# LCSL/nys-koop-lqr

Hardware: AMD Instinct MI355X
Metric: Nyström-Koopman fits/sec (K_nm build + A,B,C solve), N=1e5 m=2000 d=384 (higher is better)
Workload: dtype f64

## Files before the change

### nys_koop_lqr_amd/csrc/nk_api.hip

```cpp
#include "nk_common.h"
#include "nk_plant.h"

#include <cmath>
#include <cstdarg>
#include <cstdio>
#include <cstring>
#include <chrono>
#include <cstdlib>
#include <algorithm>
#include <condition_variable>
#include <functional>
#include <mutex>
#include <set>
#include <thread>

namespace nk {

static thread_local std::string g_err;

void set_error(const char* fmt, ...) {
  char buf[1024];
  va_list ap;
  va_start(ap, fmt);
  vsnprintf(buf, sizeof(buf), fmt, ap);
// ... 293 lines not shown
    NK_TRY(launch_gemm(ctx, false, true, len, d, m, 1.0, phi, m, mdl->W, m + p, 0.0, out + r0 * ldo, ldo));
    if (p > 0)
      NK_TRY(launch_gemm(ctx, false, true, len, d, p, 1.0, Xaug + r0 * ldx + d, ldx, mdl->W + m, m + p, 1.0,
                         out + r0 * ldo, ldo));
  }
  arena_release(ctx, mk);
  return NK_OK;
}

struct HostTrace {
  bool on;
  std::chrono::steady_clock::time_point t0, last;
  HostTrace() : on(getenv("NYSKOOP_TRACE") != nullptr) { t0 = last = std::chrono::steady_clock::now(); }
  void mark(const char* what) {
    if (!on) return;
    auto now = std::chrono::steady_clock::now();
    fprintf(stderr, "[nk trace] %-28s +%8.3f ms (total %8.3f)\n", what,
            std::chrono::duration<double, std::milli>(now - last).count(),
            std::chrono::duration<double, std::milli>(now - t0).count());
    last = now;
  }
};

static float ev_ms(nk_ctx* ctx, int a, int b) {
  float ms = 0.f;
  (void)hipEventElapsedTime(&ms, ctx->ev[a], ctx->ev[b]);
  return ms;
}

}

using namespace nk;

extern "C" {

int nk_version(void) { return NK_ABI_VERSION; }

const char* nk_last_error(void) { return g_err.c_str(); }

int nk_device_count(void) {
  int n = 0;
  if (hipGetDeviceCount(&n) != hipSuccess) {
    (void)hipGetLastError();
    return 0;
  }
  return n;
}

int nk_create(int device, nk_ctx** out) {
  NK_REQUIRE(out != nullptr, "nk_create: null output pointer");
  *out = nullptr;
  int n = nk_device_count();
  if (n <= 0) {
    set_error("no HIP device visible: libnyskoop has no CPU fallback");
    return NK_ERR_NO_DEVICE;
  }
  NK_REQUIRE(device >= 0 && device < n, "nk_create: device %d out of range (0..%d)", device, n - 1);
  NK_HIP(hipSetDevice(device));
  hipDeviceProp_t prop;
  NK_HIP(hipGetDeviceProperties(&prop, device));
  if (strncmp(prop.gcnArchName, "gfx950", 6) != 0) {
    set_error("device %d is %s; libnyskoop is built for gfx950 (MI355X) only", device, prop.gcnArchName);
    return NK_ERR_NO_DEVICE;
  }
  nk_ctx* ctx = new nk_ctx();
  ctx->device = device;
  ctx->num_cu = prop.multiProcessorCount;
  int prio_lo = 0, prio_hi = 0;
  NK_HIP(hipDeviceGetStreamPriorityRange(&prio_lo, &prio_hi));
  const int prio_mid = (prio_lo - prio_hi >= 2) ? (prio_lo + prio_hi) / 2 : prio_hi;
  NK_HIP(hipStreamCreateWithPriority(&ctx->stream_main, hipStreamNonBlocking, prio_mid));
  NK_HIP(hipStreamCreateWithPriority(&ctx->stream_side, hipStreamNonBlocking, prio_lo));
  NK_HIP(hipStreamCreateWithPriority(&ctx->stream_prep, hipStreamNonBlocking, prio_hi));
  NK_HIP(hipStreamCreateWithFlags(&ctx->stream_copy, hipStreamNonBlocking));
  NK_HIP(hipStreamCreateWithPriority(&ctx->stream_la[0], hipStreamNonBlocking, prio_hi));
  NK_HIP(hipStreamCreateWithPriority(&ctx->stream_la[1], hipStreamNonBlocking, prio_mid));
  for (int q = 0; q < 2; ++q)
    for (int i = 0; i < 4; ++i) NK_HIP(hipEventCreateWithFlags(&ctx->ev_la[q][i], hipEventDisableTiming));
  ctx->stream = ctx->stream_main;
  ctx->cur_arena = &ctx->arena;
  NK_HIP(hipEventCreateWithFlags(&ctx->ev_fork, hipEventDisableTiming));
  NK_HIP(hipEventCreateWithFlags(&ctx->ev_join, hipEventDisableTiming));
  NK_HIP(hipEventCreateWithFlags(&ctx->ev_chain, hipEventDisableTiming));
  NK_HIP(hipMalloc(reinterpret_cast<void**>(&ctx->d_info), 256));
  ctx->d_piv = reinterpret_cast<unsigned long long*>(ctx->d_info + 16);
  NK_HIP(hipMalloc(reinterpret_cast<void**>(&ctx->d_scalars), 64 * sizeof(double)));
  NK_HIP(hipHostMalloc(reinterpret_cast<void**>(&ctx->h_scalars), 64 * sizeof(double), hipHostMallocMapped | hipHostMallocCoherent));
  NK_HIP(hipHostMalloc(reinterpret_cast<void**>(&ctx->h_info), 256, hipHostMallocMapped | hipHostMallocCoherent));
  ctx->h_piv = reinterpret_cast<unsigned long long*>(ctx->h_info + 16);
  for (int i = 0; i < 16; ++i) NK_HIP(hipEventCreate(&ctx->ev[i]));
  NK_HIP(hipEventCreateWithFlags(&ctx->ev_ext, hipEventDisableTiming));
  for (int i = 0; i < 8; ++i) NK_HIP(hipEventCreateWithFlags(&ctx->ev_up[i], hipEventDisableTiming));
  const char* km = getenv("NYSKOOP_KMAT");
  ctx->kmat_mode = (km && strcmp(km, "direct") == 0) ? 1 : 0;
  const char* st = getenv("NYSKOOP_STRICT_SPD");
  ctx->strict_spd = (st && atoi(st) != 0) ? 1 : 0;
  if (const char* rp = getenv("NYSKOOP_REFINE_PIVOT")) ctx->refine_pivot = atof(rp);
  if (const char* rs = getenv("NYSKOOP_REFINE_STEPS")) ctx->refine_steps = std::max(0, atoi(rs));
  {
    std::lock_guard<std::mutex> lk(g_reg_mu);
    g_ctxs.insert(ctx);
  }
  *out = ctx;
  return NK_OK;
}

static void destroy_ctx_unregistered(nk_ctx* ctx) {
  (void)hipSetDevice(ctx->device);
  if (tl_ctx == ctx) tl_ctx = nullptr;
  group_detach(ctx);
  (void)hipStreamSynchronize(ctx->stream_main);
  (void)hipStreamSynchronize(ctx->stream_side);
  (void)hipStreamSynchronize(ctx->stream_prep);
  (void)hipStreamSynchronize(ctx->stream_copy);
  for (int q = 0; q < 2; ++q) {
    if (ctx->stream_la[q]) { (void)hipStreamSynchronize(ctx->stream_la[q]); (void)hipStreamDestroy(ctx->stream_la[q]); }
    for (int i = 0; i < 4; ++i) if (ctx->ev_la[q][i]) (void)hipEventDestroy(ctx->ev_la[q][i]);
  }
  for (auto& c : ctx->arena.chunks) (void)hipFree(c.base);
  for (auto& c : ctx->arena_side.chunks) (void)hipFree(c.base);
  (void)hipEventDestroy(ctx->ev_fork);
  (void)hipEventDestroy(ctx->ev_join);
  if (ctx->ev_chain) (void)hipEventDestroy(ctx->ev_chain);
  if (ctx->ev_ext) (void)hipEventDestroy(ctx->ev_ext);
  for (int i = 0; i < 8; ++i) if (ctx->ev_up[i]) (void)hipEventDestroy(ctx->ev_up[i]);
  (void)hipStreamDestroy(ctx->stream_side);
  (void)hipStreamDestroy(ctx->stream_prep);
  (void)hipStreamDestroy(ctx->stream_copy);
  (void)hipFree(ctx->d_info);
  for (int i = 0; i < 2; ++i) if (ctx->d_flow[i]) (void)hipFree(ctx->d_flow[i]);
  (void)hipFree(ctx->d_scalars);
  if (ctx->d_zeros) (void)hipFree(ctx->d_zeros);
  if (ctx->h_stage) (void)hipHostFree(ctx->h_stage);
  (void)hipHostFree(ctx->h_scalars);
  (void)hipHostFree(ctx->h_info);
  for (int i = 0; i < 16; ++i) (void)hipEventDestroy(ctx->ev[i]);
  (void)hipStreamDestroy(ctx->stream_main);
  delete ctx;
}

int nk_destroy(nk_ctx* ctx) {
  if (!ctx) return NK_OK;
  {
    std::lock_guard<std::mutex> lk(g_reg_mu);
    if (g_ctxs.erase(ctx) == 0) return NK_OK;
  }
  destroy_ctx_unregistered(ctx);
  return NK_OK;
}

static int model_wait_unchecked(nk_model* mdl);
static void destroy_model_unregistered(nk_model* model, bool to_pool) {
  (void)model_wait_unchecked(model);
  if (to_pool) {
    pool_give(model->device, model->bytes, model->buf);
  } else {
    (void)hipSetDevice(model->device);
    (void)hipFree(model->buf);
  }
  delete model;
}

int nk_shutdown(void) {
  tl_ctx = nullptr;
  std::set<nk_ctx*> ctxs;
  std::set<nk_model*> models;
  std::set<void*> blocks;
  {
    std::lock_guard<std::mutex> lk(g_reg_mu);
    ctxs.swap(g_ctxs);
    models.swap(g_models);
    blocks.swap(g_host_blocks);
  }
  for (nk_ctx* c : ctxs) {
    (void)hipSetDevice(c->device);
    (void)hipStreamSynchronize(c->stream_main);
    (void)hipStreamSynchronize(c->stream_side);
    (void)hipStreamSynchronize(c->stream_prep);
    (void)hipStreamSynchronize(c->stream_copy);
  }
  for (nk_model* m : models) destroy_model_unregistered(m, false);
  for (nk_ctx* c : ctxs) destroy_ctx_unregistered(c);
  pool_drain();
  for (void* b : blocks) (void)hipHostFree(b);
  return NK_OK;
}

int nk_set_compute_dtype(nk_ctx* ctx, int dtype) {
  NK_REQUIRE(ctx != nullptr && (dtype == NK_DTYPE_F64 || dtype == NK_DTYPE_F32), "nk_set_compute_dtype: bad argument");
  ctx->compute_f32 = dtype == NK_DTYPE_F32 ? 1 : 0;
  return NK_OK;
}

int nk_set_strict_spd(nk_ctx* ctx, int strict) {
  NK_REQUIRE(ctx != nullptr && strict >= 0 && strict <= 2, "nk_set_strict_spd: bad argument");
  ctx->strict_spd = strict;
  return NK_OK;
}

int nk_set_refine(nk_ctx* ctx, double pivot_ratio, int32_t steps) {
  NK_REQUIRE(ctx != nullptr && pivot_ratio >= 0.0 && pivot_ratio <= 1.0 && steps >= 0 && steps <= 8, "nk_set_refine: bad argument");
  ctx->refine_pivot = pivot_ratio;
  ctx->refine_steps = steps;
  return NK_OK;
}

// ... 2112 lines not shown
```

### nys_koop_lqr_amd/csrc/nk_common.h

```cpp
#pragma once
#include <hip/hip_runtime.h>
#include <stdint.h>
#include <stddef.h>
#include <string>
#include <vector>

#include "nyskoop.h"
#include "nk_lockstep.h"

namespace nk {

void set_error(const char* fmt, ...);

#define NK_HIP(call)                                                                         \
  do {                                                                                       \
    hipError_t e_ = (call);                                                                  \
    if (e_ != hipSuccess) {                                                                  \
      nk::set_error("%s failed: %s (%s:%d)", #call, hipGetErrorString(e_), __FILE__, __LINE__); \
      return e_ == hipErrorOutOfMemory ? NK_ERR_OOM : NK_ERR_HIP;                            \
    }                                                                                        \
  } while (0)

#define NK_TRY(call)            \
  do {                          \
    int rc_ = (call);           \
    if (rc_ != NK_OK) return rc_; \
  } while (0)

#define NK_REQUIRE(cond, ...)     \
  do {                            \
    if (!(cond)) {                \
      nk::set_error(__VA_ARGS__); \
      return NK_ERR_BAD_ARG;      \
    }                             \
  } while (0)

struct ArenaChunk {
  char* base = nullptr;
  size_t cap = 0;
  size_t off = 0;
};
struct Arena {
  std::vector<ArenaChunk> chunks;
  int cur = 0;
};
struct ArenaMark {
  int chunk;
  size_t off;
};

}

struct nk_member_state;
struct nk_ctx {
  int device = 0;
  hipStream_t stream = nullptr;
  hipStream_t stream_main = nullptr;
  hipStream_t stream_side = nullptr;
  hipStream_t stream_copy = nullptr;
  hipStream_t stream_prep = nullptr;
  nk::Arena arena;
  nk::Arena arena_side;
  nk::Arena* cur_arena = nullptr;
  hipStream_t stream_la[2] = {nullptr, nullptr};
  hipEvent_t ev_la[2][4] = {};
  int compute_f32 = 0;
  hipEvent_t ev_fork = nullptr, ev_join = nullptr, ev_chain = nullptr;
  int* d_info = nullptr;
  unsigned long long* d_piv = nullptr;
  unsigned long long* h_piv = nullptr;
  double* d_scalars = nullptr;
  double* h_scalars = nullptr;
  int* h_info = nullptr;
  double* d_zeros = nullptr;
  hipEvent_t ev[16];
  int num_cu = 256;
  int kmat_mode = 0;
  double refine_pivot = 0.0;
  int refine_steps = 2;
  int strict_spd = 0;
  hipEvent_t ev_ext = nullptr;
  hipEvent_t ev_up[8] = {};
  nk_group* group = nullptr;
  nk_member_state* gstate = nullptr;
  int* d_flow[2] = {nullptr, nullptr};
  size_t flow_words[2] = {0, 0};
  bool spline_defer_svd = false;
  bool chol_flow_off = false;
  double* h_stage = nullptr;
  size_t h_stage_bytes = 0;
};

enum { NK_MODEL_NYSTROM = 0, NK_MODEL_SPLINE = 1 };
struct nk_model {
  int device = 0;
  int32_t m = 0, d = 0, p = 0;
  int32_t ktype = 0;
  double sigma0 = 0.0;
  double jitter = 0.0;
  double* buf = nullptr;
  size_t bytes = 0;
  double *A = nullptr, *B = nullptr, *C = nullptr, *W = nullptr, *S = nullptr, *Sinv = nullptr, *Z = nullptr,
         *winv = nullptr;
  bool has_ops = false;
  int32_t kind = 0;
  hipEvent_t ev_fetch = nullptr;
};

namespace nk {

struct SideScope {
  nk_ctx* c;
  hipStream_t s0;
  Arena* a0;
  explicit SideScope(nk_ctx* ctx, hipStream_t s = nullptr) : c(ctx), s0(ctx->stream), a0(ctx->cur_arena) {
    c->stream = s ? s : c->stream_side;
    c->cur_arena = &c->arena_side;
  }
  ~SideScope() {
    c->stream = s0;
    c->cur_arena = a0;
  }
};

struct ChainOnly {
  nk_ctx* c;
  bool b0;
  explicit ChainOnly(nk_ctx* ctx) : c(ctx), b0(ctx->chol_flow_off) { c->chol_flow_off = true; }
  ~ChainOnly() { c->chol_flow_off = b0; }
};

inline int info_base(const nk_ctx* c) { return c->stream != c->stream_main ? 2 : 0; }

__device__ __forceinline__ double exp_nonpos_ca() {
  double ca = __longlong_as_double(0x3e5ade156a5dcb37LL);
  asm volatile("" : "+v"(ca));
  return ca;
}
__device__ __forceinline__ double exp_nonpos(double x, double ca_v) {
  const double k = __builtin_rint(x * __longlong_as_double(0x3ff71547652b82feLL));
  double r = __builtin_fma(__longlong_as_double((long long)0xbfe62e42fefa39efULL), k, x);
  r = __builtin_fma(__longlong_as_double((long long)0xbc7abc9e3b39803fULL), k, r);
  double p;
#define NK_EXP_STEP(c) asm("v_fma_f64 %0, %1, %2, %3" : "=v"(p) : "v"(r), "v"(p), "s"(c))
  asm("v_fma_f64 %0, %1, %2, %3" : "=v"(p) : "v"(r), "v"(ca_v), "s"(__longlong_as_double(0x3e928af3fca7ab0cLL)));
  NK_EXP_STEP(__longlong_as_double(0x3ec71dee623fde64LL));
  NK_EXP_STEP(__longlong_as_double(0x3efa01997c89e6b0LL));
  NK_EXP_STEP(__longlong_as_double(0x3f2a01a014761f6eLL));
  NK_EXP_STEP(__longlong_as_double(0x3f56c16c1852b7b0LL));
  NK_EXP_STEP(__longlong_as_double(0x3f81111111122322LL));
  NK_EXP_STEP(__longlong_as_double(0x3fa55555555502a1LL));
  NK_EXP_STEP(__longlong_as_double(0x3fc5555555555511LL));
  NK_EXP_STEP(__longlong_as_double(0x3fe000000000000bLL));
#undef NK_EXP_STEP
  p = __builtin_fma(r, p, 1.0);
  p = __builtin_fma(r, p, 1.0);
  return x < -1075.0 ? 0.0 : ldexp(p, (int)k);
}
__device__ __forceinline__ double exp_nonpos(double x) { return exp_nonpos(x, exp_nonpos_ca()); }

__host__ __device__ __forceinline__ double log_pos(double x) {
#pragma clang fp contract(off)
  const double ln2_hi = 6.93147180369123816490e-01, ln2_lo = 1.90821492927058770002e-10;
  const double Lg1 = 6.666666666666735130e-01, Lg2 = 3.999999999940941908e-01, Lg3 = 2.857142874366239149e-01,
               Lg4 = 2.222219843214978396e-01, Lg5 = 1.818357216161805012e-01, Lg6 = 1.531383769920937332e-01,
               Lg7 = 1.479819860511658591e-01;
  uint64_t bits;
  __builtin_memcpy(&bits, &x, 8);
  int32_t hx = (int32_t)(bits >> 32);
  int k = 0;
  if (hx < 0x00100000) {
    x *= 1.80143985094819840000e+16;
    k -= 54;
    __builtin_memcpy(&bits, &x, 8);
    hx = (int32_t)(bits >> 32);
  }
  k += (hx >> 20) - 1023;
  hx &= 0x000fffff;
  const int32_t i = (hx + 0x95f64) & 0x100000;
  bits = ((uint64_t)(uint32_t)(hx | (i ^ 0x3ff00000)) << 32) | (bits & 0xffffffffULL);
  __builtin_memcpy(&x, &bits, 8);
  k += i >> 20;
  const double f = x - 1.0;
  const double dk = (double)k;
  if ((0x000fffff & (2 + hx)) < 3) {
    if (f == 0.0) return k == 0 ? 0.0 : dk * ln2_hi + dk * ln2_lo;
    const double R = f * f * (0.5 - 0.33333333333333333 * f);
    return k == 0 ? f - R : dk * ln2_hi - ((R - dk * ln2_lo) - f);
  }
  const double s = f / (2.0 + f);
  const double z = s * s;
  const double w = z * z;
  const double t1 = w * (Lg2 + w * (Lg4 + w * Lg6));
  const double t2 = z * (Lg1 + w * (Lg3 + w * (Lg5 + w * Lg7)));
  const double R = t2 + t1;
  if (((hx - 0x6147a) | (0x6b851 - hx)) > 0) {
    const double hfsq = 0.5 * f * f;
    return k == 0 ? f - (hfsq - s * (hfsq + R)) : dk * ln2_hi - ((hfsq - (s * (hfsq + R) + dk * ln2_lo)) - f);
  }
  return k == 0 ? f - s * (f - R) : dk * ln2_hi - ((s * (f - R) - dk * ln2_lo) - f);
}
__host__ __device__ __forceinline__ double tps_value(double r2) {
#pragma clang fp contract(off)
  return r2 > 0.0 ? r2 * log_pos(sqrt(r2)) : 0.0;
}

nk_group* group_new(int device, int size);
void group_attach(nk_group* g, int slot, nk_ctx* c);
void group_detach(nk_ctx* c);
int group_enter(nk_ctx* c);
int group_leave(nk_ctx* c);
void group_stats(nk_ctx* c, uint64_t out[4]);
enum { CNT_CHAIN_GIVEUP = 0, CNT_JACOBI_GIVEUP = 1, CNT_RANK_TRUNCATED = 2, CNT_SQRT_RETRY = 3, CNT_REFINED = 4,
       CNT_CHOL_FLOW_GIVEUP = 5, CNT_CHOL_FLOW = 6, CNT_N = 7 };
void count_event(int which);
uint64_t read_counter(int which);
hipError_t real_stream_sync(hipStream_t s);
hipError_t real_event_sync(hipEvent_t e);

int arena_reset(nk_ctx* ctx);
ArenaMark arena_mark(nk_ctx* ctx);
void arena_release(nk_ctx* ctx, ArenaMark mk);
int arena_alloc(nk_ctx* ctx, size_t bytes, void** out);
template <typename T>
inline int arena_alloc_t(nk_ctx* ctx, size_t count, T** out) {
  return arena_alloc(ctx, count * sizeof(T), reinterpret_cast<void**>(out));
}
bool is_device_ptr(const void* p);

int launch_kmat(nk_ctx* ctx, int ktype, const double* A, int64_t lda, int64_t nA, const double* B, int64_t ldb,
                int64_t nB, int d, const double* winv, double sigma0, double* out, int64_t ldo);

enum { TRI_FULL = 0, TRI_UPPER_MIRROR = 1, TRI_LOWER = 2 };
struct GemmOpts {
  int tri = TRI_FULL;
  int splitk = 0;
};
int launch_gemm(nk_ctx* ctx, bool transA, bool transB, int64_t M, int64_t N, int64_t K, double alpha, const double* A,
                int64_t lda, const double* B, int64_t ldb, double beta, double* C, int64_t ldc,
                const GemmOpts& opts = GemmOpts(), float* ms_kernel = nullptr);

struct GemmCall {
  int64_t M = 0, N = 0, K = 0;
  double alpha = 1.0, beta = 0.0;
  const double* A = nullptr;
  const double* B = nullptr;
  double* C = nullptr;
  int64_t lda = 0, ldb = 0, ldc = 0;
  GemmOpts opts;
};
int launch_gemm_pair(nk_ctx* ctx, bool transA, bool transB, const GemmCall* calls, int ncalls);

struct TnSkip;
int launch_add_diag(nk_ctx* ctx, double* A, int64_t lda, int n, double v);
int launch_copy2d(nk_ctx* ctx, const double* src, int64_t lds, double* dst, int64_t ldd, int64_t rows, int64_t cols);
int launch_axpby2d(nk_ctx* ctx, double a, const double* X, int64_t ldx, double b, double* Y, int64_t ldy,
                   int64_t rows, int64_t cols);
int launch_scale_add_identity(nk_ctx* ctx, double a, const double* X, int64_t ldx, double c, double* Y, int64_t ldy,
                              int n, const TnSkip* skip = nullptr);
int launch_fill(nk_ctx* ctx, double* A, int64_t lda, int64_t rows, int64_t cols, double v);
int launch_frob_minus_identity(nk_ctx* ctx, const double* M, int64_t ldm, int n, double* d_out,
                               const TnSkip* skip = nullptr);
int launch_max_abs_rowsum(nk_ctx* ctx, const double* M, int64_t ldm, int n, double* d_out);
int launch_colsum_sqdiff(nk_ctx* ctx, const double* P, int64_t ldp, const double* Y, int64_t ldy, int64_t rows,
                         int cols, double* d_colsum);

int sqrtm_spd(nk_ctx* ctx, const double* P, int64_t ldp, int m, double* S, double* Sinv, int* iters, double* resid);
struct SqrtPlan {
  const double* P = nullptr;
  int64_t ldp = 0;
  int m = 0;
  double* W = nullptr;
  double* Linv = nullptr;
  double* X0 = nullptr;
  double* X0t = nullptr;
  double* d_sc = nullptr;
  ArenaMark mark{0, 0};
  bool deferred = false;
  int rc = 0, iters = 0, kmax = 0;
  double resid = 0.0;
  double lambda_min_hint = 0.0;
  bool early = false;
  int info_slot = 2;
  bool flow_gave_up = false;
  hipEvent_t pause_event = nullptr;
  int pause_step = -1;
};
constexpr int NK_SQRT_RETRY = 1;
int sqrtm_spd_coupled(nk_ctx* ctx, const double* P, int64_t ldp, int m, double* S, double* Sinv, int* iters, double* resid);
int sqrtm_prepare(nk_ctx* ctx, const double* P, int64_t ldp, int m, SqrtPlan* plan);
int sqrtm_finish(nk_ctx* ctx, SqrtPlan* plan, double* S, double* Sinv);
int sqrtm_verdict(nk_ctx* ctx, SqrtPlan* plan, int* iters, double* resid);
int cholesky_lower(nk_ctx* ctx, double* P, int64_t ldp, int m, double* Linv );
int cholesky_solve(nk_ctx* ctx, const double* L, int64_t ldl, int m, const double* Linv, double* R, int64_t ldr,
                   int nrhs);
struct CholSys {
  double* P = nullptr;
  int64_t ldp = 0;
  int m = 0;
  int extra = 0;
  bool backward = true;
  double* Linv = nullptr;
  double* pivlog = nullptr;
  double* R = nullptr;
  int64_t ldr = 0;
  int nrhs = 0;
};
int cholesky_lower_pair(nk_ctx* ctx, const CholSys* sys, int nsys);
int cholesky_lower_pair_async(nk_ctx* ctx, const CholSys* sys, int nsys);
int cholesky_check_pair(nk_ctx* ctx, const CholSys* sys, int nsys);
int cholesky_solve_pair(nk_ctx* ctx, const CholSys* sys, int nsys);
int cholesky_aug_pair_async(nk_ctx* ctx, const CholSys* sys, int nsys, hipEvent_t pause = nullptr, int pause_step = -1);
constexpr int CHOL_NB = 64;
constexpr int CHOL_WS = 2 * CHOL_NB * CHOL_NB + 8;
constexpr double CHOL_FIX_KAPPA = 8.0 * CHOL_NB;
inline int chol_fix_enabled() {
  const char* e = getenv("NYSKOOP_CHOL_FIX");
  return (e && e[0] == '0') ? 0 : ((e && e[0] == '2') ? 2 : 1);
}
bool launch_chol_trail_pair(nk_ctx* ctx, const GemmCall* calls, int ncalls, int* rc);
bool launch_chol_trail_potrf_pair(nk_ctx* ctx, const GemmCall* calls, int ncalls, const int* nb, double* const* Linv, int blk,
                                  double* const* plog, int* rc);
inline bool chol_fuse_enabled() {
  const char* e = getenv("NYSKOOP_CHOL_FUSE");
  return !(e && e[0] == '0');
}
bool chol_flow_enabled();
int cholesky_flow_pair(nk_ctx* ctx, const CholSys* sys, int nsys);
constexpr int CHOL_FLOW_GIVEUP = -0x40000000;
bool launch_chol_panel_pair(nk_ctx* ctx, const GemmCall* calls, int ncalls, int* rc);
int launch_trsm_right_lower_pair(nk_ctx* ctx, const CholSys* sys, int nsys);

struct PinvInfo {
  int rank = 0, sweeps = 0;
  bool converged = false;
  double sigma_max = 0.0, sigma_min_kept = 0.0, sigma_min = 0.0;
};
int pinv_right_divide(nk_ctx* ctx, const double* P, int64_t ldp, int m, const double* E, int64_t lde, int rows,
                      double* E_out, int64_t ldeo, double rcond, PinvInfo* info);
int cholesky_fail_flags(nk_ctx* ctx, const CholSys* sys, int nsys, int* failed , double* piv_ratio = nullptr);

int launch_lifted_step(nk_ctx* ctx, const double* G, int64_t ldg, int m, int mz, int pu, const double* z, int64_t zstride,
                       const double* u, int64_t ustride, const double* bias, double* out, int64_t ostride, int batch);

struct ChainArgs {
  const double* G = nullptr; int64_t ldg = 0; int m = 0, pu = 0;
  const double* z0 = nullptr; int64_t z0_stride = 0;
  bool lift = false;
  const double* x0 = nullptr; int64_t x0_stride = 0;
  const double* Zl = nullptr; int d = 0; const double* winv = nullptr; const double* Sinv = nullptr; int ktype = 0;
  double sigma0 = 0.0;
  const double* U = nullptr; int64_t u_stride = 0;
  const double* bias = nullptr; int64_t bias_stride = 0;
  double* Zall = nullptr; int64_t z_stride = 0;
  int T = 0, batch = 0;
};
int launch_ref_minus_traj(nk_ctx* ctx, const double* ref, int64_t ref_stride, const double* Phi, int64_t phi_stride,
                          double* D, int64_t d_stride, int steps, int m, int batch);
bool lifted_chain_ok(int m, int pu, int d_lift);
int launch_lifted_chain(nk_ctx* ctx, const ChainArgs& a);
bool lifted_chain_mw_ok(const nk_ctx* ctx, int m, int pu);
int chain_mw_workgroups(int m);
int chain_mw_group(int m, int batch);
int launch_lifted_chain_mw(nk_ctx* ctx, const ChainArgs& a);
int lifted_chain_mw_reset(nk_ctx* ctx);
int lifted_chain_mw_fetch_status(nk_ctx* ctx);
bool lifted_chain_mw_timed_out(nk_ctx* ctx, int* row, int* step, int* traj);

int plant_loop_max_m();
int launch_plant_loop(nk_ctx* ctx, const nk_model* mdl, int plant, double Ts, const double* w, const double* x0,
                      int64_t x0_stride, const double* xref, int64_t xref_stride, int steps, int batch, double* out_x,
                      int64_t ldx, double* out_u, int64_t ldu);
// ... 108 lines not shown
```

### nys_koop_lqr_amd/csrc/nk_group.hip

```cpp
#define NK_LOCKSTEP_NO_MACROS
#include "nk_common.h"

#include <algorithm>
#include <atomic>
#include <condition_variable>
#include <cstdio>
#include <cstdlib>
#include <cstring>
#include <map>
#include <mutex>
#include <unordered_map>

namespace nk {

thread_local nk_ctx* tl_ctx = nullptr;

struct TwinInfo {
  const void* twin;
  size_t bytes;
  const char* name;
};
static std::unordered_map<const void*, TwinInfo>& twin_map() {
  static std::unordered_map<const void*, TwinInfo> m;
  return m;
// ... 358 lines not shown
    const int64_t n = (int64_t)(bytes / 4);
    const int64_t blocks = (n + 1023) / 1024;
    ArgPack<const uint32_t*, uint32_t*, int64_t> pk;
    memset(static_cast<void*>(&pk), 0, sizeof(pk));
    pack_fill(pk, static_cast<const uint32_t*>(src), static_cast<uint32_t*>(dst), n);
    std::vector<uint32_t> offs;
    pack_offsets(pk, reinterpret_cast<const char*>(&pk), offs);
    (void)group_record_kernel(c, reinterpret_cast<const void*>(copy_words_kernel), dim3((unsigned)(blocks < 1 ? 1 : (blocks > 2048 ? 2048 : blocks))),
                              dim3(256), 0, &pk, sizeof(pk), offs);
    return hipSuccess;
  }
  GroupOp op;
  op.kind = OP_MEMCPY; op.dst = dst; op.src = src; op.bytes = bytes; op.mk = kind;
  st(c)->ops.push_back(op);
  return hipSuccess;
}
hipError_t x_memcpy2d_async(void* dst, size_t dpitch, const void* src, size_t spitch, size_t width, size_t height,
                            hipMemcpyKind kind, hipStream_t s) {
  nk_ctx* c = rec_ctx();
  if (!c) return hipMemcpy2DAsync(dst, dpitch, src, spitch, width, height, kind, s);
  GroupOp op;
  op.kind = OP_MEMCPY2D; op.dst = dst; op.src = src; op.dpitch = dpitch; op.spitch = spitch; op.width = width;
  op.height = height; op.mk = kind;
  st(c)->ops.push_back(op);
  return hipSuccess;
}
hipError_t x_memset_async(void* dst, int value, size_t bytes, hipStream_t s) {
  nk_ctx* c = rec_ctx();
  if (!c) return hipMemsetAsync(dst, value, bytes, s);
  GroupOp op;
  op.kind = OP_MEMSET; op.dst = dst; op.value = value; op.bytes = bytes;
  st(c)->ops.push_back(op);
  return hipSuccess;
}
hipError_t x_stream_sync(hipStream_t s) {
  nk_ctx* c = rec_ctx();
  if (!c) return hipStreamSynchronize(s);
  return group_sync(c) == NK_OK ? hipSuccess : hipErrorUnknown;
}
hipError_t x_event_sync(hipEvent_t e) {
  nk_ctx* c = rec_ctx();
  if (!c) return hipEventSynchronize(e);
  return group_sync(c) == NK_OK ? hipSuccess : hipErrorUnknown;
}
hipError_t x_event_record(hipEvent_t e, hipStream_t s) {
  if (rec_ctx()) return hipSuccess;
  return hipEventRecord(e, s);
}
hipError_t x_stream_wait_event(hipStream_t s, hipEvent_t e, unsigned flags) {
  if (rec_ctx()) return hipSuccess;
  return hipStreamWaitEvent(s, e, flags);
}
hipError_t x_event_elapsed(float* ms, hipEvent_t a, hipEvent_t b) {
  if (rec_ctx()) {
    if (ms) *ms = 0.f;
    return hipSuccess;
  }
  return hipEventElapsedTime(ms, a, b);
}

nk_group* group_new(int device, int size) {
  nk_group* g = new nk_group();
  g->device = device;
  g->members.assign((size_t)size, nullptr);
  g->live = size;
  if (hipStreamCreateWithFlags(&g->stream, hipStreamNonBlocking) != hipSuccess) { delete g; return nullptr; }
  g->tab_cap = (size_t)8 << 20;
  if (hipHostMalloc(reinterpret_cast<void**>(&g->h_tab), g->tab_cap, hipHostMallocDefault) != hipSuccess ||
      hipMalloc(reinterpret_cast<void**>(&g->d_tab), g->tab_cap) != hipSuccess) {
    if (g->h_tab) (void)hipHostFree(g->h_tab);
    (void)hipStreamDestroy(g->stream);
    delete g;
    return nullptr;
  }
  return g;
}
void group_attach(nk_group* g, int slot, nk_ctx* c) {
  g->members[(size_t)slot] = c;
  c->group = g;
  c->gstate = new nk_member_state();
}
static std::atomic<uint64_t> g_counters[CNT_N];
void count_event(int which) { if (which >= 0 && which < CNT_N) g_counters[which].fetch_add(1, std::memory_order_relaxed); }
uint64_t read_counter(int which) { return g_counters[which].load(std::memory_order_relaxed); }
hipError_t real_stream_sync(hipStream_t s) { return hipStreamSynchronize(s); }
hipError_t real_event_sync(hipEvent_t e) { return hipEventSynchronize(e); }
hipStream_t group_stream(nk_group* g) { return g->stream; }
void group_detach(nk_ctx* c) {
  nk_group* g = c->group;
  if (!g) return;
  bool last = false;
  {
    std::unique_lock<std::mutex> lk(g->mu);
    nk_member_state* s = st(c);
    if (!s->ops.empty()) (void)flush_and_sync_locked(g, std::vector<nk_ctx*>{c});
    if (s->entered) { s->entered = false; g->active--; }
    for (auto& m : g->members) if (m == c) m = nullptr;
    last = --g->live == 0;
    if (!last && g->active > 0 && g->waiting >= g->active) {
      const std::vector<nk_ctx*> ready = waiting_members(g);
      const int rc = flush_and_sync_locked(g, ready);
      release_waiters_locked(g, ready, rc);
      g->cv.notify_all();
    }
  }
  delete c->gstate;
  c->gstate = nullptr;
  c->group = nullptr;
  if (last) {
    (void)hipStreamSynchronize(g->stream);
    (void)hipFree(g->d_tab);
    (void)hipHostFree(g->h_tab);
    (void)hipStreamDestroy(g->stream);
    delete g;
  }
}
int group_enter(nk_ctx* c) {
  nk_group* g = c->group;
  if (!g) return NK_OK;
  std::lock_guard<std::mutex> lk(g->mu);
  if (!st(c)->entered) { st(c)->entered = true; g->active++; }
  return NK_OK;
}
int group_leave(nk_ctx* c) {
  nk_group* g = c->group;
  if (!g) return NK_OK;
  std::unique_lock<std::mutex> lk(g->mu);
  nk_member_state* s = st(c);
  if (!s->entered) return NK_OK;
  int rc_own = NK_OK;
  if (!s->ops.empty())
    rc_own = flush_and_sync_locked(g, std::vector<nk_ctx*>{c});
  s->entered = false;
  g->active--;
  if (g->active > 0 && g->at_align >= g->active) {
    g->at_align = 0;
    g->align_gen++;
  }
  if (g->active > 0 && g->waiting >= g->active) {
    const std::vector<nk_ctx*> ready = waiting_members(g);
    const int rc = flush_and_sync_locked(g, ready);
    release_waiters_locked(g, ready, rc);
    lk.unlock();
    g->cv.notify_all();
  }
  return rc_own;
}
void group_stats(nk_ctx* c, uint64_t out[4]) {
  nk_group* g = c->group;
  out[0] = out[1] = out[2] = out[3] = 0;
  if (!g) return;
  std::lock_guard<std::mutex> lk(g->mu);
  out[0] = g->n_flush; out[1] = g->n_launch_merged; out[2] = g->n_launch_single; out[3] = g->n_units_merged;
}

}
```

### nys_koop_lqr_amd/csrc/nk_linalg.hip

```cpp
#include "nk_common.h"

#include <algorithm>
#include <cmath>
#include <cstring>
#include <vector>

namespace nk {

__device__ __forceinline__ void add_diag_kernel_body(double* A, int64_t lda, int n, double v) {
  int i = blockIdx.x * blockDim.x + threadIdx.x;
  if (i < n) A[(int64_t)i * lda + i] += v;
}
__global__ void __launch_bounds__(256) add_diag_kernel(double* A, int64_t lda, int n, double v) { add_diag_kernel_body(A, lda, n, v); }
NK_BATCHED_TWIN(add_diag_kernel, (256), double*, int64_t, int, double)
__device__ __forceinline__ void copy2d_kernel_body(const double* __restrict__ src, int64_t lds, double* __restrict__ dst, int64_t ldd, int64_t rows, int64_t cols) {
  const int64_t total = rows * cols;
  for (int64_t e = blockIdx.x * (int64_t)blockDim.x + threadIdx.x; e < total; e += (int64_t)gridDim.x * blockDim.x) {
    const int64_t r = e / cols, c = e - r * cols;
    dst[r * ldd + c] = src[r * lds + c];
  }
}
__global__ void __launch_bounds__(256) copy2d_kernel(const double* __restrict__ src, int64_t lds, double* __restrict__ dst, int64_t ldd, int64_t rows, int64_t cols) { copy2d_kernel_body(src, lds, dst, ldd, rows, cols); }
NK_BATCHED_TWIN(copy2d_kernel, (256), const double*, int64_t, double*, int64_t, int64_t, int64_t)
__device__ __forceinline__ void axpby2d_kernel_body(double a, const double* __restrict__ X, int64_t ldx, double b, double* __restrict__ Y, int64_t ldy, int64_t rows, int64_t cols) {
// ... 831 lines not shown
  return NK_OK;
}

int cholesky_lower(nk_ctx* ctx, double* P, int64_t ldp, int m, double* Linv) {
  CholSys y;
  y.P = P; y.ldp = ldp; y.m = m; y.Linv = Linv;
  return cholesky_lower_pair(ctx, &y, 1);
}

int cholesky_solve(nk_ctx* ctx, const double* L, int64_t ldl, int m, const double* Linv, double* R, int64_t ldr,
                   int nrhs) {
  CholSys y;
  y.P = const_cast<double*>(L); y.ldp = ldl; y.m = m; y.Linv = const_cast<double*>(Linv); y.R = R; y.ldr = ldr;
  y.nrhs = nrhs;
  return cholesky_solve_pair(ctx, &y, 1);
}

__device__ __forceinline__ void tri_scale_both_kernel_body(const double* __restrict__ L, int64_t ldl, int m, const double* __restrict__ d_c, double* __restrict__ Xt, double* __restrict__ X) {
  __shared__ double tile[32][33];
  const double s = 1.0 / sqrt(d_c[0]);
  const int bx = blockIdx.x * 32, by = blockIdx.y * 32;
  const int tx = threadIdx.x & 31, ty = threadIdx.x >> 5;
  for (int r = ty; r < 32; r += 8) {
    const int i = by + r, j = bx + tx;
    double v = 0.0;
    if (i < m && j <= i) v = L[(int64_t)i * ldl + j] * s;
    if (i < m && j < m) Xt[(int64_t)i * m + j] = v;
    tile[r][tx] = v;
  }
  __syncthreads();
  for (int r = ty; r < 32; r += 8) {
    const int i = bx + r, j = by + tx;
    if (i < m && j < m) X[(int64_t)i * m + j] = tile[tx][r];
  }
}
__global__ void __launch_bounds__(256) tri_scale_both_kernel(const double* __restrict__ L, int64_t ldl, int m, const double* __restrict__ d_c, double* __restrict__ Xt, double* __restrict__ X) { tri_scale_both_kernel_body(L, ldl, m, d_c, Xt, X); }
NK_BATCHED_TWIN(tri_scale_both_kernel, (256), const double*, int64_t, int, const double*, double*, double*)

int sqrtm_prepare(nk_ctx* ctx, const double* P, int64_t ldp, int m, SqrtPlan* plan) {
  plan->P = P; plan->ldp = ldp; plan->m = m;
  plan->mark = arena_mark(ctx);
  const size_t mm = (size_t)m * m;
  const int nblk = (m + CHOL_NB - 1) / CHOL_NB;
  NK_TRY(arena_alloc_t(ctx, 2 * mm, &plan->W));
  NK_TRY(arena_alloc_t(ctx, (size_t)nblk * CHOL_WS, &plan->Linv));
  NK_TRY(arena_alloc_t(ctx, mm, &plan->X0));
  NK_TRY(arena_alloc_t(ctx, mm, &plan->X0t));
  NK_TRY(arena_alloc_t(ctx, (size_t)8, &plan->d_sc));
  NK_TRY(launch_max_abs_rowsum(ctx, P, ldp, m, plan->d_sc));
  {
    const ArenaMark mk = arena_mark(ctx);
    const int blocks = grid_for((int64_t)m * m, ctx->num_cu);
    double* partial = nullptr;
    NK_TRY(arena_alloc_t(ctx, (size_t)2 * blocks, &partial));
    hipLaunchKernelGGL(sumsq_trace_partial_kernel, dim3(blocks), dim3(256), 0, ctx->stream, P, ldp, m, partial, blocks);
    hipLaunchKernelGGL(sum_partials_kernel, dim3(1), dim3(256), 0, ctx->stream, partial, blocks, plan->d_sc + 1);
    hipLaunchKernelGGL(sum_partials_kernel, dim3(1), dim3(256), 0, ctx->stream, partial + blocks, blocks, plan->d_sc + 2);
    NK_HIP(hipGetLastError());
    arena_release(ctx, mk);
  }
  NK_HIP(hipMemcpyAsync(ctx->h_scalars + 12, plan->d_sc, 3 * sizeof(double), hipMemcpyDeviceToHost, ctx->stream));
  NK_HIP(hipEventRecord(ctx->ev[11], ctx->stream));
  double* E = plan->W + mm;
  NK_TRY(launch_copy2d(ctx, P, ldp, plan->W, m, m, m));
  NK_TRY(launch_fill(ctx, E, m, m, m, 0.0));
  NK_TRY(launch_add_diag(ctx, E, m, m, 1.0));
  CholSys y;
  y.P = plan->W; y.ldp = m; y.m = m; y.extra = m; y.backward = false; y.Linv = plan->Linv;
  NK_TRY(cholesky_aug_pair_async(ctx, &y, 1, plan->pause_event, plan->pause_step));
  {
    const ArenaMark mk = arena_mark(ctx);
    const int blocks = grid_for((int64_t)m * m, ctx->num_cu);
    double* partial = nullptr;
    NK_TRY(arena_alloc_t(ctx, (size_t)2 * blocks, &partial));
    hipLaunchKernelGGL(sumsq_trace_partial_kernel, dim3(blocks), dim3(256), 0, ctx->stream, E, (int64_t)m, m, partial, blocks);
    hipLaunchKernelGGL(sum_partials_kernel, dim3(1), dim3(256), 0, ctx->stream, partial, blocks, plan->d_sc + 3);
    NK_HIP(hipGetLastError());
    arena_release(ctx, mk);
  }
  const int tb = (m + 31) / 32;
  hipLaunchKernelGGL(tri_scale_both_kernel, dim3(tb, tb), dim3(256), 0, ctx->stream, plan->W, (int64_t)m, m, plan->d_sc,
                     plan->X0t, plan->X0);
  NK_HIP(hipGetLastError());
  return NK_OK;
}

__device__ __forceinline__ void ns_flag_kernel_body(const double* __restrict__ partial, int count, int m, int step, double* __restrict__ state) {
  __shared__ double sh[4];
  double s = 0.0;
  for (int i = threadIdx.x; i < count; i += blockDim.x) s += partial[i];
  s = wave_sum(s);
  if ((threadIdx.x & 63) == 0) sh[threadIdx.x >> 6] = s;
  __syncthreads();
  if (threadIdx.x == 0) {
    const double r = sqrt((sh[0] + sh[1] + sh[2] + sh[3]) / m);
    state[2] = r;
    if (state[0] == 0.0 && r < 1e-7) {
      state[0] = (double)(step + 1);
      state[1] = r;
    }
  }
}
__global__ void __launch_bounds__(256) ns_flag_kernel(const double* __restrict__ partial, int count, int m, int step, double* __restrict__ state) { ns_flag_kernel_body(partial, count, m, step, state); }
NK_BATCHED_TWIN(ns_flag_kernel, (256), const double*, int, int, int, double*)

static int sqrtm_polar_products(nk_ctx* ctx, SqrtPlan* plan, const double* Q, double* scratch, double c, double* S,
                                double* Sinv, const double* Q_even = nullptr, const double* select = nullptr) {
  const int m = plan->m;
  const size_t mm = (size_t)m * m;
  double* Linv_full = scratch;
  NK_TRY(launch_transpose(ctx, plan->W + mm, m, Linv_full, m, m, m));
  TnProblem pr[2];
  pr[0].A = Q; pr[0].B = plan->X0; pr[0].C = S; pr[0].lda = pr[0].ldb = pr[0].ldc = m; pr[0].M = pr[0].N = m;
  pr[0].alpha = std::sqrt(c);
  pr[0].ktrim = KTRIM_B_UPPER;
  pr[1].ktrim = KTRIM_A_LOWER;
  pr[1].A = Linv_full; pr[1].B = Q; pr[1].C = Sinv; pr[1].lda = pr[1].ldb = pr[1].ldc = m; pr[1].M = pr[1].N = m;
  pr[0].A_even = Q_even;
  pr[1].B_even = Q_even;
  TnSkip sel;
  sel.select = select;
  if (tn_fast_ok(pr[0]) && tn_fast_ok(pr[1]) && m >= 128) {
    NK_TRY(launch_gemm_tn_multi(ctx, pr, 2, m, 0, nullptr, true, select ? &sel : nullptr));
  } else {
    NK_TRY(launch_gemm(ctx, true, false, m, m, m, pr[0].alpha, Q, m, plan->X0, m, 0.0, S, m));
    NK_TRY(launch_gemm(ctx, true, false, m, m, m, 1.0, Linv_full, m, Q, m, 0.0, Sinv, m));
  }
  return NK_OK;
}

int sqrtm_finish(nk_ctx* ctx, SqrtPlan* plan, double* S, double* Sinv) {
  const int m = plan->m;
  const size_t mm = (size_t)m * m;
  const int ib = info_base(ctx);
  plan->deferred = false;
  plan->info_slot = ib;
  plan->rc = NK_OK; plan->iters = 0; plan->resid = 0.0;
  plan->early = plan->lambda_min_hint > 0.0 && m >= 1024 && m % 2 == 0;
  double c, sumsq, trace, linv2 = 0.0;
  if (plan->early) {
    NK_HIP(hipEventSynchronize(ctx->ev[11]));
    c = ctx->h_scalars[12]; sumsq = ctx->h_scalars[13]; trace = ctx->h_scalars[14];
    if (!(c > 0.0) || !std::isfinite(c)) plan->early = false;
  }
  if (!plan->early) {
    NK_HIP(hipMemcpyAsync(ctx->h_scalars, plan->d_sc, 4 * sizeof(double), hipMemcpyDeviceToHost, ctx->stream));
    NK_HIP(hipMemcpyAsync(ctx->h_info + ib, ctx->d_info + ib, sizeof(int), hipMemcpyDeviceToHost, ctx->stream));
    NK_HIP(hipStreamSynchronize(ctx->stream));
    c = ctx->h_scalars[0]; sumsq = ctx->h_scalars[1]; trace = ctx->h_scalars[2]; linv2 = ctx->h_scalars[3];
  }
  if (!plan->early && ctx->h_info[ib] == CHOL_FLOW_GIVEUP) {
    count_event(CNT_CHOL_FLOW_GIVEUP);
    arena_release(ctx, plan->mark);
    ChainOnly chain(ctx);
    SqrtPlan again;
    NK_TRY(sqrtm_prepare(ctx, plan->P, plan->ldp, m, &again));
    const int rc = sqrtm_finish(ctx, &again, S, Sinv);
    *plan = again;
    return rc;
  }
  if (!plan->early &&
      (ctx->h_info[ib] != 0 || !(c > 0.0) || !std::isfinite(c) || !(linv2 > 0.0) || !std::isfinite(linv2))) {
    arena_release(ctx, plan->mark);
    plan->rc = sqrtm_spd_coupled(ctx, plan->P, plan->ldp, m, S, Sinv, &plan->iters, &plan->resid);
    return plan->rc;
  }
  double *Xa = nullptr, *Xta = nullptr, *Xb = nullptr, *Xtb = nullptr, *M = nullptr, *T = nullptr;
  NK_TRY(arena_alloc_t(ctx, mm, &Xa));
  NK_TRY(arena_alloc_t(ctx, mm, &Xta));
  NK_TRY(arena_alloc_t(ctx, mm, &Xb));
  NK_TRY(arena_alloc_t(ctx, mm, &Xtb));
  NK_TRY(arena_alloc_t(ctx, mm, &M));
  NK_TRY(arena_alloc_t(ctx, mm, &T));
  double a_lo = 1.0, b_hi = 1.0;
  {
    const double fro = std::sqrt(sumsq) / c, tr = trace / c;
    const double lam1 = fro < 1.0 ? fro : 1.0;
    if (m > 1 && tr > lam1) a_lo = (tr - lam1) / (m - 1);
    else a_lo = tr / m * 1e-2;
    if (!(a_lo > 0.0) || !std::isfinite(a_lo)) a_lo = 1e-12;
    if (a_lo > 1.0) a_lo = 1.0;
  }
  auto p3 = [](double x) { return x * (3.0 - x) * (3.0 - x) * 0.25; };
  auto advance = [&](double s2, double& a, double& b) {
    const double xa = s2 * a, xb = s2 * b;
    const double lo = p3(xa) < p3(xb) ? p3(xa) : p3(xb);
    b = (xa <= 1.0 && xb >= 1.0) ? 1.0 : (p3(xa) > p3(xb) ? p3(xa) : p3(xb));
    a = lo < b ? lo : b;
  };
  GemmOpts sym;
  sym.tri = TRI_UPPER_MIRROR;
  const double* X = plan->X0;
  const double* Xt = plan->X0t;
  double *Xn = Xa, *Xtn = Xta;
  TnProblem probe;
  probe.A = Xta; probe.B = T; probe.C = Xa; probe.lda = probe.ldb = probe.ldc = m; probe.M = probe.N = m;
  const bool fast = m >= 128 && tn_fast_ok(probe);
  const bool queued = fast && m >= 1024;
  if (plan->early && !queued) {
    set_error("sqrtm: internal: early queueing needs the LDS-DMA path");
    return NK_ERR_BAD_ARG;
  }

  if (queued) {
    double s2s[128];
    bool checks[128];
    int kmax = 0;
    {
      double ta = plan->early ? 0.9 * plan->lambda_min_hint / c : 0.5 / (c * linv2), tb = 1.0;
      if (ta > a_lo) ta = a_lo;
      const double a_sched = std::pow(a_lo, 0.8) * std::pow(ta, 0.2);
      double a = a_sched, b = b_hi;
      int kconv = -1;
      for (int k = 0; k < 100; ++k) {
        if (kconv < 0 && ta >= 1.0 - 1e-9 && tb <= 1.0 + 1e-9) kconv = k;
        checks[k] = a >= 0.5;
        const double s2 = 3.0 / (a + std::sqrt(a * b) + b);
        s2s[k] = s2;
        advance(s2, a, b);
        advance(s2, ta, tb);
        if (kconv >= 0 && k >= kconv + 1) { kmax = k + 1; break; }
      }
      if (kmax == 0) kmax = 100;
    }
    double* state = plan->d_sc + 5;
    NK_HIP(hipMemsetAsync(state, 0, 3 * sizeof(double), ctx->stream));
    double* rpart = nullptr;
    {
      const size_t mt = (size_t)(m + 127) / 128;
      const size_t need = std::max((size_t)grid_for((int64_t)m * m, ctx->num_cu), mt * (mt + 1) / 2 * 8);
      NK_TRY(arena_alloc_t(ctx, need, &rpart));
    }
    for (int k = 0; k < kmax; ++k) {
      TnSkip skip;
      skip.state = state; skip.step = k;
      int npart = 0;
      if (k == 0) {
        NK_TRY(launch_transpose(ctx, plan->P, plan->ldp, M, m, m, m));
        NK_TRY(launch_axpby2d(ctx, 0.5 / c, plan->P, plan->ldp, 0.5 / c, M, m, m, m));
      } else {
        const double s2k = s2s[k], sck = std::sqrt(s2k);
        TnProblem pm;
        pm.A = X; pm.B = X; pm.C = M; pm.lda = pm.ldb = pm.ldc = m; pm.M = pm.N = m; pm.tri = TRI_UPPER_MIRROR;
        pm.Caff = T; pm.aff_a = -0.5 * s2k * sck; pm.aff_c = 1.5 * sck;
        TnSkip skip_m = skip;
        skip_m.resid_partials = rpart; skip_m.resid_count = &npart;
        NK_TRY(launch_gemm_tn_multi(ctx, &pm, 1, m, 0, nullptr, true, &skip_m));
      }
      if (checks[k]) {
        if (npart == 0) {
          npart = grid_for((int64_t)m * m, ctx->num_cu);
          hipLaunchKernelGGL(frob_mi_partial_kernel, dim3(npart), dim3(256), 0, ctx->stream, M, (int64_t)m, m, rpart,
                             skip.state, skip.step);
        }
        hipLaunchKernelGGL(ns_flag_kernel, dim3(1), dim3(256), 0, ctx->stream, rpart, npart, m, k, state);
        NK_HIP(hipGetLastError());
      }
      if (k == 0) {
        const double s2 = s2s[0], sc = std::sqrt(s2);
        NK_TRY(launch_scale_add_identity(ctx, -0.5 * s2 * sc, M, m, 1.5 * sc, T, m, m, &skip));
      }
      TnProblem pr;
      pr.A = Xt; pr.B = T; pr.C = Xn; pr.lda = pr.ldb = pr.ldc = m; pr.M = pr.N = m; pr.Ct = Xtn; pr.ldct = m;
      NK_TRY(launch_gemm_tn_multi(ctx, &pr, 1, m, 1, nullptr, true, &skip));
      X = Xn; Xt = Xtn;
      Xn = (Xn == Xa) ? Xb : Xa;
      Xtn = (Xtn == Xta) ? Xtb : Xta;
    }
    NK_TRY(sqrtm_polar_products(ctx, plan, Xa, T, c, S, Sinv, Xb, state));
    NK_HIP(hipMemcpyAsync(ctx->h_scalars + 8, state, 3 * sizeof(double), hipMemcpyDeviceToHost, ctx->stream));
    if (plan->early)
      NK_HIP(hipMemcpyAsync(ctx->h_info + ib, ctx->d_info + ib, sizeof(int), hipMemcpyDeviceToHost, ctx->stream));
    plan->deferred = true;
    plan->kmax = kmax;
    arena_release(ctx, plan->mark);
    return NK_OK;
  }

  const int maxit = 100;
  double r = 1e300;
  int it = 0;
  bool ok = false;
  for (; it < maxit; ++it) {
    if (it == 0) {
      NK_TRY(launch_transpose(ctx, plan->P, plan->ldp, M, m, m, m));
      NK_TRY(launch_axpby2d(ctx, 0.5 / c, plan->P, plan->ldp, 0.5 / c, M, m, m, m));
    } else {
      NK_TRY(launch_gemm(ctx, true, false, m, m, m, 1.0, X, m, X, m, 0.0, M, m, sym));
    }
    const bool check = a_lo >= 0.5 || it + 2 >= maxit;
    if (check) {
      NK_TRY(launch_frob_minus_identity(ctx, M, m, m, ctx->d_scalars));
      NK_HIP(hipMemcpyAsync(ctx->h_scalars, ctx->d_scalars, sizeof(double), hipMemcpyDeviceToHost, ctx->stream));
      NK_HIP(hipEventRecord(ctx->ev[10], ctx->stream));
    }
    const double s2 = 3.0 / (a_lo + std::sqrt(a_lo * b_hi) + b_hi);
    const double sc = std::sqrt(s2);
    advance(s2, a_lo, b_hi);
    NK_TRY(launch_scale_add_identity(ctx, -0.5 * s2 * sc, M, m, 1.5 * sc, T, m, m));
    if (fast) {
      TnProblem pr;
      pr.A = Xt; pr.B = T; pr.C = Xn; pr.lda = pr.ldb = pr.ldc = m; pr.M = pr.N = m; pr.Ct = Xtn; pr.ldct = m;
      NK_TRY(launch_gemm_tn_multi(ctx, &pr, 1, m, 0));
    } else {
      NK_TRY(launch_gemm(ctx, true, false, m, m, m, 1.0, Xt, m, T, m, 0.0, Xn, m));
      NK_TRY(launch_transpose(ctx, Xn, m, Xtn, m, m, m));
    }
    X = Xn; Xt = Xtn;
    Xn = (Xn == Xa) ? Xb : Xa;
    Xtn = (Xtn == Xta) ? Xtb : Xta;
    if (check) {
      NK_HIP(hipEventSynchronize(ctx->ev[10]));
      r = std::sqrt(ctx->h_scalars[0] / m);
      if (!std::isfinite(r)) break;
      if (r < 1e-7) {
        ok = true;
        ++it;
        break;
      }
    }
  }
  plan->iters = it;
  plan->resid = r;
  NK_TRY(x_align());
  if (!ok) {
    set_error("sqrtm: Newton-Schulz did not converge (residual %g after %d iterations)", r, it);
    arena_release(ctx, plan->mark);
    plan->rc = NK_ERR_NO_CONVERGENCE;
    return plan->rc;
  }
  NK_TRY(sqrtm_polar_products(ctx, plan, X, T, c, S, Sinv));
  arena_release(ctx, plan->mark);
  return NK_OK;
}

int sqrtm_verdict(nk_ctx* ctx, SqrtPlan* plan, int* iters, double* resid) {
  if (plan->deferred) {
    const double flag = ctx->h_scalars[8];
    plan->deferred = false;
    const int word = ctx->h_info[plan->info_slot];
    if (plan->early && (word != 0 || flag == 0.0 || !std::isfinite(ctx->h_scalars[10]))) {
      plan->flow_gave_up = word == CHOL_FLOW_GIVEUP;
      if (plan->flow_gave_up) count_event(CNT_CHOL_FLOW_GIVEUP);
      plan->iters = plan->kmax;
      plan->resid = ctx->h_scalars[10];
      plan->rc = NK_SQRT_RETRY;
    } else if (flag == 0.0 || !std::isfinite(ctx->h_scalars[10])) {
      plan->iters = plan->kmax;
      plan->resid = ctx->h_scalars[10];
      plan->rc = NK_ERR_NO_CONVERGENCE;
      set_error("sqrtm: Newton-Schulz did not converge (residual %g after %d iterations)", plan->resid, plan->kmax);
    } else {
      plan->iters = (int)flag;
      plan->resid = ctx->h_scalars[9];
      plan->rc = NK_OK;
    }
  }
  if (iters) *iters = plan->iters;
  if (resid) *resid = plan->resid;
  return plan->rc;
}

int sqrtm_spd(nk_ctx* ctx, const double* P, int64_t ldp, int m, double* S, double* Sinv, int* iters, double* resid) {
  SqrtPlan plan;
  NK_TRY(sqrtm_prepare(ctx, P, ldp, m, &plan));
  NK_TRY(sqrtm_finish(ctx, &plan, S, Sinv));
  NK_HIP(hipStreamSynchronize(ctx->stream));
  return sqrtm_verdict(ctx, &plan, iters, resid);
}

}
```

Measured before the change: 24.47.

## Trim Newton-Schulz sqrtm iterations using host-side early exit and refined budget

The deferred Newton-Schulz matrix square root previously enqueued a fixed, conservatively scheduled number of GEMM steps, using device-side skip flags to no-op the converged ones. In lean mode the host queues a few blind steps, then reads back a spectral bound to recompute a tighter iteration budget. It then polls the convergence flag through a mapped host mirror, staying two steps behind, so it can stop enqueueing steps once converged. This is meant to cut launch and skipped-kernel overhead. The cost is extra host syncs that may stall the pipeline, and it is disabled during graph capture.

New measurement: 24.47. No clear change (-0.0%).

```diff
diff --git a/nys_koop_lqr_amd/csrc/nk_api.hip b/nys_koop_lqr_amd/csrc/nk_api.hip
--- a/nys_koop_lqr_amd/csrc/nk_api.hip
+++ b/nys_koop_lqr_amd/csrc/nk_api.hip
@@ -399,6 +399,8 @@
   NK_HIP(hipEventCreateWithFlags(&ctx->ev_fork, hipEventDisableTiming));
   NK_HIP(hipEventCreateWithFlags(&ctx->ev_join, hipEventDisableTiming));
   NK_HIP(hipEventCreateWithFlags(&ctx->ev_chain, hipEventDisableTiming));
+  NK_HIP(hipEventCreateWithFlags(&ctx->ev_sqrt, hipEventDisableTiming));
+  for (int i = 0; i < 8; ++i) NK_HIP(hipEventCreateWithFlags(&ctx->ev_ns[i], hipEventDisableTiming));
   NK_HIP(hipMalloc(reinterpret_cast<void**>(&ctx->d_info), 256));
   ctx->d_piv = reinterpret_cast<unsigned long long*>(ctx->d_info + 16);
   NK_HIP(hipMalloc(reinterpret_cast<void**>(&ctx->d_scalars), 64 * sizeof(double)));
@@ -439,6 +441,8 @@
   (void)hipEventDestroy(ctx->ev_fork);
   (void)hipEventDestroy(ctx->ev_join);
   if (ctx->ev_chain) (void)hipEventDestroy(ctx->ev_chain);
+  if (ctx->ev_sqrt) (void)hipEventDestroy(ctx->ev_sqrt);
+  for (int i = 0; i < 8; ++i) if (ctx->ev_ns[i]) (void)hipEventDestroy(ctx->ev_ns[i]);
   if (ctx->ev_ext) (void)hipEventDestroy(ctx->ev_ext);
   for (int i = 0; i < 8; ++i) if (ctx->ev_up[i]) (void)hipEventDestroy(ctx->ev_up[i]);
   (void)hipStreamDestroy(ctx->stream_side);
diff --git a/nys_koop_lqr_amd/csrc/nk_common.h b/nys_koop_lqr_amd/csrc/nk_common.h
--- a/nys_koop_lqr_amd/csrc/nk_common.h
+++ b/nys_koop_lqr_amd/csrc/nk_common.h
@@ -66,6 +66,8 @@
   hipEvent_t ev_la[2][4] = {};
   int compute_f32 = 0;
   hipEvent_t ev_fork = nullptr, ev_join = nullptr, ev_chain = nullptr;
+  hipEvent_t ev_sqrt = nullptr;
+  hipEvent_t ev_ns[8] = {};
   int* d_info = nullptr;
   unsigned long long* d_piv = nullptr;
   unsigned long long* h_piv = nullptr;
@@ -212,8 +214,9 @@
 int group_leave(nk_ctx* c);
 void group_stats(nk_ctx* c, uint64_t out[4]);
 enum { CNT_CHAIN_GIVEUP = 0, CNT_JACOBI_GIVEUP = 1, CNT_RANK_TRUNCATED = 2, CNT_SQRT_RETRY = 3, CNT_REFINED = 4,
-       CNT_CHOL_FLOW_GIVEUP = 5, CNT_CHOL_FLOW = 6, CNT_N = 7 };
+       CNT_CHOL_FLOW_GIVEUP = 5, CNT_CHOL_FLOW = 6, CNT_NS_STEPS = 7, CNT_N = 8 };
 void count_event(int which);
+void count_events(int which, uint64_t n);
 uint64_t read_counter(int which);
 hipError_t real_stream_sync(hipStream_t s);
 hipError_t real_event_sync(hipEvent_t e);
@@ -281,6 +284,7 @@
   double resid = 0.0;
   double lambda_min_hint = 0.0;
   bool early = false;
+  bool lean = false;
   int info_slot = 2;
   bool flow_gave_up = false;
   hipEvent_t pause_event = nullptr;
@@ -288,6 +292,7 @@
 };
 constexpr int NK_SQRT_RETRY = 1;
 int sqrtm_spd_coupled(nk_ctx* ctx, const double* P, int64_t ldp, int m, double* S, double* Sinv, int* iters, double* resid);
+bool sqrt_lean_enabled();
 int sqrtm_prepare(nk_ctx* ctx, const double* P, int64_t ldp, int m, SqrtPlan* plan);
 int sqrtm_finish(nk_ctx* ctx, SqrtPlan* plan, double* S, double* Sinv);
 int sqrtm_verdict(nk_ctx* ctx, SqrtPlan* plan, int* iters, double* resid);
diff --git a/nys_koop_lqr_amd/csrc/nk_group.hip b/nys_koop_lqr_amd/csrc/nk_group.hip
--- a/nys_koop_lqr_amd/csrc/nk_group.hip
+++ b/nys_koop_lqr_amd/csrc/nk_group.hip
@@ -464,6 +464,7 @@
 }
 static std::atomic<uint64_t> g_counters[CNT_N];
 void count_event(int which) { if (which >= 0 && which < CNT_N) g_counters[which].fetch_add(1, std::memory_order_relaxed); }
+void count_events(int which, uint64_t n) { if (which >= 0 && which < CNT_N) g_counters[which].fetch_add(n, std::memory_order_relaxed); }
 uint64_t read_counter(int which) { return g_counters[which].load(std::memory_order_relaxed); }
 hipError_t real_stream_sync(hipStream_t s) { return hipStreamSynchronize(s); }
 hipError_t real_event_sync(hipEvent_t e) { return hipEventSynchronize(e); }
diff --git a/nys_koop_lqr_amd/csrc/nk_linalg.hip b/nys_koop_lqr_amd/csrc/nk_linalg.hip
--- a/nys_koop_lqr_amd/csrc/nk_linalg.hip
+++ b/nys_koop_lqr_amd/csrc/nk_linalg.hip
@@ -937,10 +937,20 @@
   hipLaunchKernelGGL(tri_scale_both_kernel, dim3(tb, tb), dim3(256), 0, ctx->stream, plan->W, (int64_t)m, m, plan->d_sc,
                      plan->X0t, plan->X0);
   NK_HIP(hipGetLastError());
-  return NK_OK;
-}
-
-__device__ __forceinline__ void ns_flag_kernel_body(const double* __restrict__ partial, int count, int m, int step, double* __restrict__ state) {
+  plan->lean = plan->lambda_min_hint > 0.0 && sqrt_lean_enabled() && !ctx_recording(ctx);
+  if (plan->lean) {
+    NK_HIP(hipMemcpyAsync(ctx->h_scalars + 15, plan->d_sc + 3, sizeof(double), hipMemcpyDeviceToHost, ctx->stream));
+    NK_HIP(hipEventRecord(ctx->ev_sqrt, ctx->stream));
+  }
+  return NK_OK;
+}
+
+bool sqrt_lean_enabled() {
+  const char* e = getenv("NYSKOOP_SQRT_LEAN");
+  return !(e && e[0] == '0');
+}
+
+__device__ __forceinline__ void ns_flag_kernel_body(const double* __restrict__ partial, int count, int m, int step, double* __restrict__ state, double* __restrict__ mirror) {
   __shared__ double sh[4];
   double s = 0.0;
   for (int i = threadIdx.x; i < count; i += blockDim.x) s += partial[i];
@@ -954,10 +964,11 @@
       state[0] = (double)(step + 1);
       state[1] = r;
     }
-  }
-}
-__global__ void __launch_bounds__(256) ns_flag_kernel(const double* __restrict__ partial, int count, int m, int step, double* __restrict__ state) { ns_flag_kernel_body(partial, count, m, step, state); }
-NK_BATCHED_TWIN(ns_flag_kernel, (256), const double*, int, int, int, double*)
+    if (mirror) mirror[0] = state[0];
+  }
+}
+__global__ void __launch_bounds__(256) ns_flag_kernel(const double* __restrict__ partial, int count, int m, int step, double* __restrict__ state, double* __restrict__ mirror) { ns_flag_kernel_body(partial, count, m, step, state, mirror); }
+NK_BATCHED_TWIN(ns_flag_kernel, (256), const double*, int, int, int, double*, double*)
 
 static int sqrtm_polar_products(nk_ctx* ctx, SqrtPlan* plan, const double* Q, double* scratch, double c, double* S,
                                 double* Sinv, const double* Q_even = nullptr, const double* select = nullptr) {
@@ -984,6 +995,10 @@
   return NK_OK;
 }
 
+constexpr int NS_LEAN_BLIND = 4;
+constexpr int NS_LEAN_AHEAD = 2;
+constexpr int NS_LEAN_RING = 8;
+
 int sqrtm_finish(nk_ctx* ctx, SqrtPlan* plan, double* S, double* Sinv) {
   const int m = plan->m;
   const size_t mm = (size_t)m * m;
@@ -1061,9 +1076,11 @@
     double s2s[128];
     bool checks[128];
     int kmax = 0;
+    double ta_sched = 0.0;
     {
       double ta = plan->early ? 0.9 * plan->lambda_min_hint / c : 0.5 / (c * linv2), tb = 1.0;
       if (ta > a_lo) ta = a_lo;
+      ta_sched = ta;
       const double a_sched = std::pow(a_lo, 0.8) * std::pow(ta, 0.2);
       double a = a_sched, b = b_hi;
       int kconv = -1;
@@ -1078,6 +1095,17 @@
       }
       if (kmax == 0) kmax = 100;
     }
+    auto budget_for = [&](double ta) {
+      double tb = 1.0;
+      int kconv = -1;
+      for (int k = 0; k < kmax; ++k) {
+        if (kconv < 0 && ta >= 1.0 - 1e-9 && tb <= 1.0 + 1e-9) kconv = k;
+        advance(s2s[k], ta, tb);
+        if (kconv >= 0 && k >= kconv + 1) return k + 1;
+      }
+      return kmax;
+    };
+    const bool lean = plan->early && plan->lean;
     double* state = plan->d_sc + 5;
     NK_HIP(hipMemsetAsync(state, 0, 3 * sizeof(double), ctx->stream));
     double* rpart = nullptr;
@@ -1086,7 +1114,7 @@
       const size_t need = std::max((size_t)grid_for((int64_t)m * m, ctx->num_cu), mt * (mt + 1) / 2 * 8);
       NK_TRY(arena_alloc_t(ctx, need, &rpart));
     }
-    for (int k = 0; k < kmax; ++k) {
+    auto queue_step = [&](int k) -> int {
       TnSkip skip;
       skip.state = state; skip.step = k;
       int npart = 0;
@@ -1108,8 +1136,10 @@
           hipLaunchKernelGGL(frob_mi_partial_kernel, dim3(npart), dim3(256), 0, ctx->stream, M, (int64_t)m, m, rpart,
                              skip.state, skip.step);
         }
-        hipLaunchKernelGGL(ns_flag_kernel, dim3(1), dim3(256), 0, ctx->stream, rpart, npart, m, k, state);
+        hipLaunchKernelGGL(ns_flag_kernel, dim3(1), dim3(256), 0, ctx->stream, rpart, npart, m, k, state,
+                           lean ? ctx->h_scalars + 24 : (double*)nullptr);
         NK_HIP(hipGetLastError());
+        if (lean) NK_HIP(hipEventRecord(ctx->ev_ns[k % NS_LEAN_RING], ctx->stream));
       }
       if (k == 0) {
         const double s2 = s2s[0], sc = std::sqrt(s2);
@@ -1121,7 +1151,29 @@
       X = Xn; Xt = Xtn;
       Xn = (Xn == Xa) ? Xb : Xa;
       Xtn = (Xtn == Xta) ? Xtb : Xta;
-    }
+      return NK_OK;
+    };
+    const int kblind = lean ? std::min(kmax, NS_LEAN_BLIND) : kmax;
+    if (lean) ctx->h_scalars[24] = 0.0;
+    for (int k = 0; k < kblind; ++k) NK_TRY(queue_step(k));
+    if (kblind < kmax) {
+      NK_HIP(hipEventSynchronize(ctx->ev_sqrt));
+      const double l2 = ctx->h_scalars[15];
+      double ta = 0.5 / (c * l2);
+      if (l2 > 0.0 && std::isfinite(l2) && ta > 0.0 && std::isfinite(ta) && ta > ta_sched) {
+        if (ta > a_lo) ta = a_lo;
+        kmax = std::max(kblind, budget_for(ta));
+      }
+    }
+    for (int k = kblind; k < kmax; ++k) {
+      const int seen = k - NS_LEAN_AHEAD;
+      if (seen >= 0 && checks[seen]) {
+        NK_HIP(hipEventSynchronize(ctx->ev_ns[seen % NS_LEAN_RING]));
+        if (ctx->h_scalars[24] != 0.0) { kmax = k; break; }
+      }
+      NK_TRY(queue_step(k));
+    }
+    count_events(CNT_NS_STEPS, (uint64_t)kmax);
     NK_TRY(sqrtm_polar_products(ctx, plan, Xa, T, c, S, Sinv, Xb, state));
     NK_HIP(hipMemcpyAsync(ctx->h_scalars + 8, state, 3 * sizeof(double), hipMemcpyDeviceToHost, ctx->stream));
     if (plan->early)
@@ -1177,6 +1229,7 @@
   }
   plan->iters = it;
   plan->resid = r;
+  count_events(CNT_NS_STEPS, (uint64_t)std::min(it + (ok ? 0 : 1), maxit));
   NK_TRY(x_align());
   if (!ok) {
     set_error("sqrtm: Newton-Schulz did not converge (residual %g after %d iterations)", r, it);
```
